# gotaku6629/CTC

Hardware: AMD Instinct MI355X
Metric: ctc_samples_per_sec (higher is better)
Workload: dtype f32; 1 GPU; NoBlankCTC B=256 T=150 C=158 S<=20 fp32 (BASELINE configs[1]); variant=noblank, per_gpu_batch=256, global_batch=256, T=150, C=158, S=20, parallelism=dp1 (batch-sharded), launch=graph, graph_steps=50, step=fused loss+grad launch + scale_grad launch (loss.backward(), grad_out=1)

## Files before the change

### __graft_entry__.py

```python
import os
import sys

ROOT = os.path.dirname(os.path.abspath(__file__))
if ROOT not in sys.path:
    sys.path.insert(0, ROOT)


def build():
    from ctc_amd import build as b
    so = b.build()
    b.build_fault()
    try:
        b.build_host_ext()
    except Exception as e:
        print("build: the optional C++ autograd node was not built (%s: %s)" % (type(e).__name__, str(e).splitlines()[0][:200]))
    b.build_occupant()
    from oracle import ctc_c
    ctc_c.build()
    import ctc_amd
    from ctc_amd import _lib
    _lib.load()
    assert os.path.exists(so) and ctc_amd.SO_PATH == so


def smoke():
    import numpy as np
# ... 23 lines not shown
```

### ctc_amd/csrc/binary.hip

```cpp
#include <cstdlib>
#include <type_traits>

#include "lattice.hpp"
#include "launch.hpp"

namespace ctc {

struct BinaryParams {
    const float *x;
    int64_t st, sb;
    const float *y;
    const int64_t *in_len, *tgt_len;
    int T, B, C, S, SP, CP;
    int stop;
    float loss_scale, grad_scale;
    float *nll, *loss, *grad;
    float *gamma;
    unsigned *counter;
};

constexpr int kBinThreads = 1024;
constexpr int kBinWaves = kBinThreads / kWave;

struct BinarySmem {
    float *em, *al, *be, *dummy, *ys, *drow;
    __device__ BinarySmem(float *base, int T, int SP, int S, int CP)
    {
        em = base + kPrefetch * SP;
        al = em + (size_t)(T + kPrefetch) * SP;
        be = al + (size_t)T * SP;
        dummy = be + (size_t)T * SP;
        ys = dummy + 8;
        drow = ys + (size_t)S * CP;
// ... 939 lines not shown
                         const int64_t *in_len, const int64_t *tgt_len, int T, int B, int C, int S, float loss_scale,
                         float grad_scale, float *nll, float *loss, float *grad, float *gamma, void *workspace,
                         const BinarySwitches &sw)
{
    if (!x || !y || !in_len || !tgt_len || !nll || !(loss || gamma) || !workspace) return CTC_AMD_ERR_BAD_ARGUMENT;
    if (T < 1 || B < 1 || C < 1 || S < 1) return CTC_AMD_ERR_BAD_ARGUMENT;
    p.x = static_cast<const float *>(x);
    p.st = stride_t; p.sb = stride_b; p.y = y;
    p.in_len = in_len; p.tgt_len = tgt_len;
    p.T = T; p.B = B; p.C = C; p.S = S;
    p.stop = sw.stop < 0 ? sw.stop : 0;
    p.loss_scale = loss_scale; p.grad_scale = grad_scale;
    p.nll = nll; p.loss = gamma ? reinterpret_cast<float *>(static_cast<char *>(workspace) + 32) : loss;
    p.grad = gamma ? nullptr : grad; p.gamma = gamma;
    p.counter = static_cast<unsigned *>(workspace);
    return 0;
}

struct BinaryQuery {
    int T, B, C, S, dtype;
    bool want_gamma;
    BinarySwitches sw;
};
enum BinaryFamily { kBinaryUnsupported = 0, kBinaryFlow, kBinaryPipe, kBinaryMfma, kBinaryFused };
struct BinaryPlan {
    int family, K, SP, ch, wt, Tpad, pd, grid;
    size_t lds;
};
static int binary_row_pitch(int C) { return C | 1; }

// ... 25 lines not shown
    BinaryPlan pl = {};
    pl.family = kBinaryFused; pl.K = K; pl.SP = SP; pl.grid = q.B;
    pl.lds = binary_smem_bytes(q.T, SP, q.S, binary_row_pitch(q.C));
    return pl.lds <= kMaxLds ? pl : BinaryPlan{};
}

static int binary_launch(const BinaryPlan &pl, int dtype, BinaryParams &p, hipStream_t s)
{
    const dim3 grid(pl.grid), block(kBinThreads);
    p.SP = pl.SP; p.CP = binary_row_pitch(p.C);
    auto workers = [&](auto wt, auto gamma, auto elem) {
        constexpr bool WT = decltype(wt)::value != 0, GAMMA = decltype(gamma)::value;
        using E = typename decltype(elem)::type;
        if (pl.family == kBinaryFlow)
            return with_constant<1, 2, 3>(pl.ch, [&](auto ch) {
                return launch<binary_flow_kernel<decltype(ch)::value, WT, GAMMA, E>>(grid, block, pl.lds, s, p, pl.pd);
            });
        return with_constant<1, 2, 3, 4>(pl.ch, [&](auto ch) {
            return launch<binary_pipe_kernel<decltype(ch)::value, WT, GAMMA, E>>(grid, block, pl.lds, s, p, pl.pd);
        });
    };
    switch (pl.family) {
        case kBinaryFlow:
        case kBinaryPipe:
            if (p.gamma) return with_logit_elem(dtype, [&](auto elem) { return workers(std::true_type(), std::true_type(), elem); });
            return with_constant<0, 1>(pl.wt, [&](auto wt) { return workers(wt, std::false_type(), LogitElem<float>()); });
        case kBinaryMfma:
            return with_constant<1, 2, 4>(pl.K, [&](auto k) {
                return with_constant<1, 2, 3, 4>(pl.ch, [&](auto ch) {
                    return with_constant<0, 1>(pl.wt, [&](auto wt) {
// ... 62 lines not shown
```

### ctc_amd/csrc/binary_flow.hpp

```cpp
#pragma once

typedef __bf16 bf16x8 __attribute__((ext_vector_type(8)));
typedef unsigned u32x4 __attribute__((ext_vector_type(4)));

#ifndef CTC_FLOW_TILE_WAVES
#define CTC_FLOW_TILE_WAVES 4
#endif
constexpr int kFlowTileWaves = CTC_FLOW_TILE_WAVES;
constexpr int kFlowFirstWorker = 2 + kFlowTileWaves;
constexpr int kFlowWorkers = kBinWaves - kFlowFirstWorker;
constexpr int kFlowRounds = (80 + kFlowWorkers - 1) / kFlowWorkers;
static_assert(kFlowRounds % 2 == 0, "two rounds per gradient group");
constexpr int kFlowGroups = kFlowRounds / 2;
constexpr int kFlowMaxT = 2 * kFlowWorkers * kFlowRounds;
constexpr int kFlowMaxTiles = kFlowMaxT / 16;
constexpr int kFlowFlags = 64;
constexpr int kFlowYRows = (65 + kFlowFirstWorker - 1) / kFlowFirstWorker;

__host__ __device__ inline int flow_yp(int C) { return (C + 31) / 32 * 32 + 8; }
__host__ __device__ inline size_t flow_y_floats(int SP, int C, int PD)
{
    const size_t halfs = (size_t)(SP + 1) * flow_yp(C);
    return (((size_t)SP * PD + 3) & ~(size_t)3) + (((halfs + 1) / 2 + 3) & ~(size_t)3);
}

struct BinaryFlowSmem {
    float *em, *al, *be, *dummy, *q, *zrow, *ys, *dimg;
    unsigned short *y16;
    int *prog, *fail, *tile, *done, *ystage;
    __device__ BinaryFlowSmem(float *base, int T, int SP, int PD, int C)
    {
        em = base + kPrefetch * SP;
        al = em + (size_t)(T + kPrefetch) * SP;
        be = al + (size_t)T * SP;
        dummy = be + (size_t)T * SP;
        int *f = reinterpret_cast<int *>(dummy);
        prog = f + 4;
        fail = f + 6;
        tile = f + 8;
        done = f + 20;
        ystage = f + 32;
        q = dummy + kFlowFlags;
        zrow = q + ((T + 7) & ~3);
        ys = zrow + 64;
        y16 = reinterpret_cast<unsigned short *>(ys + (((size_t)SP * PD + 3) & ~(size_t)3));
        dimg = ys + flow_y_floats(SP, C, PD);
    }
};

static size_t binary_flow_smem_bytes(int T, int SP, int PD, int C)
{
    return ((size_t)(3 * T + 2 * kPrefetch) * SP + kFlowFlags + ((T + 7) & ~3) + 64 + flow_y_floats(SP, C, PD) + (size_t)(T + 1) * PD) * 4;
}

__device__ __forceinline__ void split3_bf16(const float (&f)[8], u32x4 &t0, u32x4 &t1, u32x4 &t2)
{
// ... 78 lines not shown
                for (int j = 0; j < CH; ++j) {
                    const int c = lane + 64 * j;
                    yv[i][j] = (l < p.S && c < p.C) ? yb[l * p.C + c] : 0.f;
                }
            }
        }
    }
    if (tid < kFlowFlags) sm.dummy[tid] = 0.f;
    if (tid >= 128 && tid < 192) sm.zrow[tid - 128] = 0.f;
    for (int i = tid; i < kPrefetch * p.SP; i += kBinThreads) {
        sm.em[i - kPrefetch * p.SP] = kNeg;
        sm.em[p.T * p.SP + i] = kNeg;
    }
    __syncthreads();
    const ScalarLengths lens(p.in_len + b, p.tgt_len + b);

    auto six = [&](const int *f, int equals) -> bool {
        return __builtin_amdgcn_ballot_w64(lane < kFlowFirstWorker && *(lds_cvint *)(f + (lane < kFlowFirstWorker ? lane : 0)) == equals) != 0;
    };
    bool exact = true;
    auto wait_y = [&]() -> bool {
        int spins = 0;
        while (six(sm.ystage, 0)) {
            if (++spins >= (1 << 20)) return false;
            __builtin_amdgcn_s_sleep(1);
        }
        exact = !six(sm.ystage, 2);
        lds_order();
        return true;
    };
// ... 6 lines not shown
#pragma unroll
                for (int j = 0; j < CH; ++j) {
                    const int c = lane + 64 * j;
                    const unsigned bits = __builtin_bit_cast(unsigned, yv[i][j]);
                    inexact = inexact || (bits & 0xffffu) != 0;
                    if (c < YP) sm.y16[l * YP + c] = (unsigned short)(bits >> 16);
                    if (l < p.SP && c < PD) sm.ys[l * PD + c] = yv[i][j];
                }
            }
        }
        lds_order();
        sm.ystage[w] = __builtin_amdgcn_ballot_w64(inexact) == 0 ? 1 : 2;
    }
    int64_t Tb64, L64;
    lens.get(Tb64, L64);
    const bool ok = L64 >= 1 && L64 <= p.S && Tb64 >= L64 && Tb64 <= p.T;
    const int Tb = ok ? (int)Tb64 : 0, L = ok ? (int)L64 : 0;
    const float invC = 1.0f / (float)p.C;
    const float inv2 = invC * kLog2e;
    const float gs = p.grad_scale * invC;
    stamp(p, 1);

    bool starved = false;
    bool have_lse = false;
    float c2 = 0.f;
    const unsigned voff = 4u * lane;
    const int lane_l = lane < p.SP ? lane : 0;
    const bool in_l = lane < L;
    const float ninf = -__builtin_inff();
    int c_tt[kFlowGroups][4], c_tl[kFlowGroups][4], c_hi[kFlowGroups], c_lo[kFlowGroups];
// ... 116 lines not shown
                if (tl[k] >= 0)
                    p.gamma[((int64_t)b * p.T + tl[k]) * p.S + lane] = starved ? __builtin_nanf("") : pe[k] * __builtin_amdgcn_rcpf(sum[k]);
        }
    };
    auto elem = [&](int uu, int jg, unsigned slow4, auto &&P, bool own = false) {
        int tt[4], tl[4], t_hi, t_lo;
        rows_of(uu, jg, tt, tl, t_hi, t_lo, own);
        if (starved) raise_status(p.counter, kStatusBinaryStarved);
        if constexpr (GAMMA) {
#pragma unroll
            for (int i = 0; i < 4; ++i)
                if (tt[i] >= 0 && tl[i] < 0 && lane < p.S) p.gamma[((int64_t)b * p.T + tt[i]) * p.S + lane] = 0.f;
            return;
        }
        lds_order();
        f32x4 acc[CH];
#pragma unroll
        for (int j = 0; j < CH; ++j) acc[j] = f32x4{0.f, 0.f, 0.f, 0.f};
        if (t_hi >= 0) {
            {
                const int ti = tl[lane & 3];
                const float *arow = ti >= 0 ? sm.be + ti * p.SP : sm.zrow;
                const float *yrow = sm.ys + lane;
                auto operands = [&](int l0, float4 &fa, float (&fy)[4][CH]) {
                    fa = *reinterpret_cast<const float4 *>(arow + (l0 < p.SP ? l0 : 0));
#pragma unroll
                    for (int i = 0; i < 4; ++i)
#pragma unroll
                        for (int j = 0; j < CH; ++j) fy[i][j] = yrow[(l0 + i < p.SP ? l0 + i : p.SP - 1) * PD + 64 * j];
                };
// ... 5 lines not shown
                        for (int j = 0; j < CH; ++j) acc[j] = __builtin_amdgcn_mfma_f32_4x4x1f32(fav[i], fy[i][j], acc[j], 0, 0, 0);
                };
                float4 fa0, fa1;
                float fy0[4][CH], fy1[4][CH];
                operands(0, fa0, fy0);
                for (int l0 = 0; l0 < L; l0 += 8) {
                    operands(l0 + 4, fa1, fy1);
                    contract(fa0, fy0);
                    if (l0 + 4 < L) {
                        operands(l0 + 8, fa0, fy0);
                        contract(fa1, fy1);
                    }
                }
            }
        }
        if (!starved && slow4 == 0 && tl[0] >= 0 && tl[1] >= 0 && tl[2] >= 0 && tl[3] >= 0) {
#pragma unroll
            for (int i = 0; i < 4; ++i) {
                float *g = p.grad + ((int64_t)tl[i] * p.B + b) * p.C;
                bin_row_base_settled(g);
#pragma unroll
                for (int j = 0; j < CH; ++j) {
                    const float pr = P(i & 1, i >> 1, j);
                    if (j < CH - 1 || lane + 64 * j < p.C) bin_store_col<WT>(g, voff, j, __builtin_fmaf(pr, gs, -acc[j][i]));
                }
            }
            return;
        }
#pragma unroll
        for (int i = 0; i < 4; ++i) {
            if (tt[i] < 0) continue;
            float *g = p.grad + ((int64_t)tt[i] * p.B + b) * p.C;
            bin_row_base_settled(g);
            const int slot = 2 * (i & 1) + (i >> 1);
            if (tl[i] < 0 || starved) {
                const float fill = starved ? __builtin_nanf("") : 0.f;
#pragma unroll
                for (int j = 0; j < CH; ++j)
                    if (j < CH - 1 || lane + 64 * j < p.C) bin_store_col<WT>(g, voff, j, fill);
            } else if ((slow4 >> slot) & 1) {
#pragma unroll
                for (int j = 0; j < CH; ++j) {
                    const float pr = P(i & 1, i >> 1, j);
                    const float pq = pr * (1.0f - pr);
                    const float gv = __builtin_fmaf(pr, gs, -acc[j][i]) * (pq * __builtin_amdgcn_rcpf(fmaxf(pq, 1e-12f)));
                    if (j < CH - 1 || lane + 64 * j < p.C) bin_store_col<WT>(g, voff, j, gv);
                }
            } else {
#pragma unroll
                for (int j = 0; j < CH; ++j) {
                    const float pr = P(i & 1, i >> 1, j);
                    if (j < CH - 1 || lane + 64 * j < p.C) bin_store_col<WT>(g, voff, j, __builtin_fmaf(pr, gs, -acc[j][i]));
                }
            }
        }
    };

    if (w < 2) {
        if (w == 1 && !p.grad && !GAMMA) return;
        __builtin_amdgcn_s_setprio(3);
        bool starved = false;
        if (Tb > 0) {
            int known = -1;
            auto ready = [&](int i) {
                while (known < i && !starved) {
                    const int t = w == 0 ? known + 1 : Tb - 2 - known;
                    const int m = t >> 4;
// ... 351 lines not shown
```

### ctc_amd/csrc/common.hpp

```cpp
#pragma once
#include <hip/hip_runtime.h>
#include <stdint.h>

#if !defined(CTC_AMD_EXPERIMENTS) &&                                                                            \
    (defined(CTC_X_NOSTATUS) || defined(CTC_X_NOREDUCE) || defined(CTC_X_NORETURN) || defined(CTC_X_NOCHAIN) || \
     defined(CTC_X_NOPRIO) || defined(CTC_X_NOREAD) || defined(CTC_X_NOWRITE) ||                                 \
     defined(CTC_X_WMASK) || defined(CTC_X_NOPROG) || defined(CTC_X_NORENORM) ||                                \
     defined(CTC_X_ROWDPP) || defined(CTC_X_SCALAR_STEP) || defined(CTC_X_NO_POOL_GATHER) || defined(CTC_X_FLOW_NO_GPRIO) || defined(CTC_X_FLOW_NOEXP) || defined(CTC_X_FLOW_NO_DELEGATE) || defined(CTC_X_FLOW_DELEGATE_OWN) || \
     defined(CTC_FLOW_TILE_WAVES))
#error "CTC_X_* experiment switches need -DCTC_AMD_EXPERIMENTS (A/B builds only, never the product library)"
#endif

namespace ctc {

constexpr int kWave = 64;
constexpr float kNeg = -10000000000000.0f;
constexpr float kInfeasible = 1.0e12f;
constexpr float kMasked = -1.0e30f;
__device__ __forceinline__ float masked_floor(float e) { return e < kMasked ? kMasked : e; }

struct LaneStates { int K, SP; };
inline LaneStates lane_states(int S)
{
    int K = 1;
// ... 254 lines not shown

struct ScalarLengths {
    int64_t a, b;
    __device__ __forceinline__ ScalarLengths() : a(0), b(0) {}
    __device__ __forceinline__ ScalarLengths(const int64_t *pa, const int64_t *pb)
    {
        typedef const __attribute__((address_space(4))) int64_t const_i64;
        a = *(const_i64 *)(uintptr_t)pa;
        b = *(const_i64 *)(uintptr_t)pb;
    }
    __device__ __forceinline__ void get(int64_t &va, int64_t &vb) const
    {
        va = a;
        vb = b;
    }
};

__device__ __forceinline__ void bce_logs(float x, float &p, float &lp, float &lq)
{
    p = 1.0f / (1.0f + expf(-x));
    lp = fmaxf(logf(p), -100.0f);
    lq = fmaxf(logf(1.0f - p), -100.0f);
}

template <typename P>
__device__ __forceinline__ void stamp(const P &p, int slot)
{
    if (CTC_DIAG(p) >= 0 || CTC_DIAG(p) <= -100) return;
    if (blockIdx.x == 0 && wave_id() == -CTC_DIAG(p) - 1 && lane_id() == 0) {
        unsigned long long *o = reinterpret_cast<unsigned long long *>(p.counter) + 8 + 2 * slot;
// ... 120 lines not shown
```

### ctc_amd/csrc/launch.hpp

```cpp
#pragma once
#include <hip/hip_runtime.h>

#include <atomic>
#include <cstdlib>
#include <type_traits>

#include "../../include/ctc_amd.h"

namespace ctc {

constexpr size_t kMaxLds = 160 * 1024;
constexpr size_t kDefaultDynLds = 64 * 1024;
constexpr int kMaxDevices = 64;

inline bool within_memory_side_cache(size_t bytes, int T, int B, int C) { return bytes * T * B * C <= ((size_t)230 << 20); }

inline int current_device()
{
    int dev = -1;
    if (hipGetDevice(&dev) != hipSuccess || dev < 0 || dev >= kMaxDevices) return -1;
    return dev;
}

inline int device_cus()
// ... 47 lines not shown
{
    if (smem > kDefaultDynLds) {
        static std::atomic<bool> granted[kMaxDevices];
        const int dev = current_device();
        if (dev < 0 || !granted[dev].load(std::memory_order_relaxed)) {
            hipError_t e = hipFuncSetAttribute(reinterpret_cast<const void *>(kern),
                                               hipFuncAttributeMaxDynamicSharedMemorySize, (int)kMaxLds);
            if (e != hipSuccess) return (int)e;
            if (dev >= 0) granted[dev].store(true, std::memory_order_relaxed);
        }
    }
    hipLaunchKernelGGL(kern, grid, block, smem, stream, args...);
    return (int)hipGetLastError();
}

}
```

### ctc_amd/csrc/noblank.hip

```cpp
#include <type_traits>

#include "lattice.hpp"
#include "launch.hpp"

namespace ctc {

struct NoblankParams {
    const float *x;
    int64_t st, sb;
    const void *lab;
    int lab64;
    const int64_t *in_len, *tgt_len;
    int T, B, C, S, SP;
    int stop;
    float loss_scale, grad_scale;
    float *nll, *loss, *grad;
    float *gamma;
    float *lattice;
    int64_t slab;
    unsigned *counter;
    int next_round;
    float ls_a, ls_b;
    int koff;
};

__device__ __forceinline__ NoblankParams opaque_params(NoblankParams q)
{
#define CTC_OPQ(f) asm volatile("" : "+s"(q.f))
    CTC_OPQ(x); CTC_OPQ(st); CTC_OPQ(sb); CTC_OPQ(lab); CTC_OPQ(lab64); CTC_OPQ(in_len); CTC_OPQ(tgt_len);
    CTC_OPQ(T); CTC_OPQ(B); CTC_OPQ(C); CTC_OPQ(S); CTC_OPQ(SP); CTC_OPQ(stop); CTC_OPQ(loss_scale); CTC_OPQ(grad_scale);
    CTC_OPQ(nll); CTC_OPQ(loss); CTC_OPQ(grad); CTC_OPQ(gamma); CTC_OPQ(lattice); CTC_OPQ(slab); CTC_OPQ(counter);
    CTC_OPQ(next_round); CTC_OPQ(ls_a); CTC_OPQ(ls_b); CTC_OPQ(koff);
#undef CTC_OPQ
    return q;
}

#ifndef CTC_NOBLANK_THREADS
#define CTC_NOBLANK_THREADS 1024
#endif
constexpr int kThreads = CTC_NOBLANK_THREADS;
constexpr int kWaves = kThreads / kWave;
constexpr int kRows = 160 / kWaves;
constexpr int kRowsPerPass = kWaves * kRows;

struct NoblankSmem {
    float *em, *al, *be, *mx, *ls, *dummy;
    int *cnt, *lab, *nxt, *dup, *inv;
// ... 338 lines not shown
    const size_t stride = (size_t)gridDim.x * blockDim.x;
    const size_t i = (size_t)blockIdx.x * blockDim.x + threadIdx.x;
    size_t done = 0;
    if ((reinterpret_cast<uintptr_t>(g) & 7) == 0) {
        wt_u2 *g4 = reinterpret_cast<wt_u2 *>(g);
        const size_t n4 = n / 4;
        const f2_t s2 = {s, s};
        for (size_t k = i; k < n4; k += stride) {
            wt_u2 v = g4[k];
            v.x = r16_narrow2<E>(r16_widen2<E>(v.x) * s2);
            v.y = r16_narrow2<E>(r16_widen2<E>(v.y) * s2);
            g4[k] = v;
        }
        done = n4 * 4;
    }
    for (size_t k = done + i; k < n; k += stride) g[k] = (E)((float)g[k] * s);
}


struct NoblankSwitches {
    bool no_pipe, no_xr, no_r16, no_ps, km;
    bool nograd;
    int stop;
};
static const NoblankSwitches &noblank_switches()
{
    static const NoblankSwitches sw = {diag_env("CTC_AMD_NOPIPE") != 0, diag_env("CTC_AMD_NOXR") != 0,
                                       diag_env("CTC_AMD_NOR16") != 0,  diag_env("CTC_AMD_NOPS") != 0,
                                       diag_env("CTC_AMD_KM") != 0,     diag_env("CTC_AMD_DEBUG_NOGRAD") != 0,
                                       diag_env("CTC_AMD_DEBUG_STOP")};
    return sw;
// ... 10 lines not shown
    const NoblankSizes z = noblank_sizes(T, C, S);
    char *ws = static_cast<char *>(workspace);
    p.x = static_cast<const float *>(x); p.st = stride_t; p.sb = stride_b;
    p.lab = labels; p.lab64 = labels_i64;
    p.in_len = in_len; p.tgt_len = tgt_len;
    p.T = T; p.B = B; p.C = C; p.S = S; p.SP = z.SP;
    p.stop = sw.stop;
    p.loss_scale = loss_scale; p.grad_scale = grad_scale;
    p.nll = nll; p.loss = gamma ? reinterpret_cast<float *>(ws + 32) : loss;
    p.grad = sw.nograd ? nullptr : static_cast<float *>(grad);
    p.gamma = gamma;
    p.counter = static_cast<unsigned *>(workspace);
    p.lattice = z.glb ? reinterpret_cast<float *>(ws + 256 + acc_list_bytes(B)) : nullptr;
    p.slab = z.glb ? (int64_t)noblank_lattice_floats(T, z.SP) : 0;
    p.next_round = 0; p.koff = 0;
    const bool smooth = label_smoothing >= 0.f;
    p.ls_b = smooth ? (1.f - label_smoothing) / (float)C : 0.f;
    p.ls_a = smooth ? label_smoothing - p.ls_b : 1.f;
    return 0;
}

struct NoblankQuery {
    int T, B, C, S;
    int dtype;
    int64_t st, sb;
    unsigned x_low, grad_low;
    bool want_grad, want_gamma, smooth;
    int cus;
    NoblankSwitches sw;
};
// ... 73 lines not shown
}

static int noblank_launch(const NoblankPlan &pl, int dtype, NoblankParams &p, hipStream_t s)
{
    const dim3 grid(pl.grid), block(kThreads);
    p.next_round = pl.next_round; p.koff = pl.koff;
    switch (pl.family) {
        case kNoblankR16:
            return with_row_chunks(pl.n4, pl.n2, [&](auto n4, auto n2) {
                return with_constant<0, 1>(pl.nt, [&](auto nt) {
                    return with_constant<CTC_AMD_BF16, CTC_AMD_F16, CTC_AMD_F32>(dtype, [&](auto dt) {
                        using E = std::conditional_t<decltype(dt)::value == CTC_AMD_BF16, __bf16,
                                                     std::conditional_t<decltype(dt)::value == CTC_AMD_F16, _Float16, float>>;
                        constexpr int A = decltype(n4)::value, Bq = decltype(n2)::value;
                        constexpr bool NT = decltype(nt)::value != 0;
                        if constexpr (4 * A + 2 * Bq <= 12)
                            if (pl.ps) return launch<noblank_r16_kernel<A, Bq, NT, true, E>>(grid, block, pl.lds, s, p);
                        return launch<noblank_r16_kernel<A, Bq, NT, false, E>>(grid, block, pl.lds, s, p);
                    });
                });
            });
#ifdef CTC_AMD_DIAGNOSTICS
        case kNoblankKm:
            return with_row_chunks(pl.n4, pl.n2, [&](auto n4, auto n2) {
                return with_constant<0, 1>(pl.nt, [&](auto nt) {
                    return launch<noblank_km_kernel<decltype(n4)::value, decltype(n2)::value, decltype(nt)::value != 0>>(
                        grid, block, pl.lds, s, p);
                });
            });
#endif
        case kNoblankXr:
        case kNoblankPipelined:
            return with_constant<1, 2, 3, 4>(pl.ch, [&](auto ch) {
// ... 68 lines not shown
                                                  const int64_t *in_len, const int64_t *tgt_len,
                                                  int T, int B, int C, int S, float label_smoothing,
                                                  float loss_scale, float grad_scale,
                                                  float *nll, float *loss, float *grad,
                                                  void *workspace, void *stream)
{
    if (!(label_smoothing >= 0.f && label_smoothing <= 1.f)) return CTC_AMD_ERR_BAD_ARGUMENT;
    return noblank_run(x, stride_t, stride_b, labels, labels_i64, in_len, tgt_len, T, B, C, S, loss_scale, grad_scale,
                       nll, loss, grad, workspace, stream, label_smoothing);
}

extern "C" int ctc_amd_scale_grad(float *grad, const float *grad_out, size_t n, void *stream)
{
    if (!grad || !grad_out) return CTC_AMD_ERR_BAD_ARGUMENT;
    if (n == 0) return 0;
    hipLaunchKernelGGL(scale_grad_kernel, scale_grad_grid(n), dim3(256), 0,
                       static_cast<hipStream_t>(stream), grad, grad_out, n);
    return (int)hipGetLastError();
}

extern "C" int ctc_amd_noblank_loss_grad_typed(const void *x, int x_dtype, int64_t stride_t, int64_t stride_b,
                                               const void *labels, int labels_i64,
                                               const int64_t *in_len, const int64_t *tgt_len,
                                               int T, int B, int C, int S, float label_smoothing,
                                               float loss_scale, float grad_scale,
                                               float *nll, float *loss, void *grad,
                                               void *workspace, void *stream)
{
    if (x_dtype != CTC_AMD_F32 && x_dtype != CTC_AMD_BF16 && x_dtype != CTC_AMD_F16) return CTC_AMD_ERR_BAD_ARGUMENT;
    if (label_smoothing != label_smoothing || label_smoothing > 1.f) return CTC_AMD_ERR_BAD_ARGUMENT;
    return noblank_run(x, stride_t, stride_b, labels, labels_i64, in_len, tgt_len, T, B, C, S, loss_scale, grad_scale,
                       nll, loss, grad, workspace, stream, label_smoothing < 0.f ? -1.f : label_smoothing, x_dtype);
}

extern "C" int ctc_amd_scale_grad_typed(void *grad, int dtype, const float *grad_out, size_t n, void *stream)
{
    if (dtype == CTC_AMD_F32) return ctc_amd_scale_grad(static_cast<float *>(grad), grad_out, n, stream);
    if ((dtype != CTC_AMD_BF16 && dtype != CTC_AMD_F16) || !grad || !grad_out) return CTC_AMD_ERR_BAD_ARGUMENT;
    if (n == 0) return 0;
    if (dtype == CTC_AMD_BF16)
        hipLaunchKernelGGL(scale_grad_lowp_kernel<__bf16>, scale_grad_grid(n), dim3(256), 0,
                           static_cast<hipStream_t>(stream), static_cast<__bf16 *>(grad), grad_out, n);
    else
        hipLaunchKernelGGL(scale_grad_lowp_kernel<_Float16>, scale_grad_grid(n), dim3(256), 0,
                           static_cast<hipStream_t>(stream), static_cast<_Float16 *>(grad), grad_out, n);
    return (int)hipGetLastError();
}

extern "C" int ctc_amd_noblank_posteriors(const float *x, int64_t stride_t, int64_t stride_b,
                                          const void *labels, int labels_i64,
                                          const int64_t *in_len, const int64_t *tgt_len,
                                          int T, int B, int C, int S,
                                          float *nll, float *gamma,
                                          void *workspace, void *stream)
// ... 5 lines not shown

extern "C" int ctc_amd_noblank_posteriors_typed(const void *x, int x_dtype, int64_t stride_t, int64_t stride_b,
                                                const void *labels, int labels_i64,
                                                const int64_t *in_len, const int64_t *tgt_len,
                                                int T, int B, int C, int S,
                                                float *nll, float *gamma,
                                                void *workspace, void *stream)
{
    if (x_dtype != CTC_AMD_F32 && x_dtype != CTC_AMD_BF16 && x_dtype != CTC_AMD_F16) return CTC_AMD_ERR_BAD_ARGUMENT;
    if (!gamma) return CTC_AMD_ERR_BAD_ARGUMENT;
    return noblank_run(x, stride_t, stride_b, labels, labels_i64, in_len, tgt_len, T, B, C, S, 0.f, 0.f, nll, nullptr,
                       nullptr, workspace, stream, -1.f, x_dtype, gamma);
}

#ifdef CTC_AMD_DIAGNOSTICS
extern "C" int ctc_amd_debug_chain_probe(int T, int SP, int waves_alive, int grid, void *out, void *stream, int mode,
                                         int chain_b)
{
    using namespace ctc;
    NoblankParams p = {};
    p.T = T; p.SP = SP; p.S = SP; p.B = grid; p.C = 32;
    p.stop = -77;
    p.counter = reinterpret_cast<unsigned *>(static_cast<unsigned long long *>(out) + 8);
    const size_t smem = r16_smem_bytes(T, SP, 158);
    return launch<r16_chain_probe_kernel>(dim3(grid), dim3(kThreads), smem, static_cast<hipStream_t>(stream), p,
                                          static_cast<unsigned long long *>(out), waves_alive, mode, chain_b);
}

extern "C" int ctc_amd_debug_noblank_plan(int T, int B, int C, int S, int dtype, int64_t stride_t, int64_t stride_b,
                                          unsigned x_low, unsigned grad_low, int want_grad, int want_gamma, int smooth,
// ... 14 lines not shown
```

### ctc_amd/csrc/noblank_r16.hpp

```cpp
#pragma once

namespace ctc {

typedef float f2_t __attribute__((ext_vector_type(2)));

#define CTC_ROW16(OP)                                                                   \
    "s_nop 1\n\t" OP " %0, %0, %0 quad_perm:[1,0,3,2] row_mask:0xf bank_mask:0xf\n\t"   \
    "s_nop 1\n\t" OP " %0, %0, %0 quad_perm:[2,3,0,1] row_mask:0xf bank_mask:0xf\n\t"   \
    "s_nop 1\n\t" OP " %0, %0, %0 row_half_mirror row_mask:0xf bank_mask:0xf\n\t"       \
    "s_nop 1\n\t" OP " %0, %0, %0 row_mirror row_mask:0xf bank_mask:0xf\n\t"            \
    "s_nop 1"
__device__ __forceinline__ void row16_allmax(float &v) { asm volatile(CTC_ROW16("v_max_f32_dpp") : "+v"(v)); }
__device__ __forceinline__ void row16_allsum(float &v) { asm volatile(CTC_ROW16("v_add_f32_dpp") : "+v"(v)); }
__device__ __forceinline__ void row16_allmax(int &v) { asm volatile(CTC_ROW16("v_max_i32_dpp") : "+v"(v)); }

constexpr int kR16Pad = 2 * kPrefetch + 1;
#ifndef CTC_R16_BLOCK
#define CTC_R16_BLOCK 16
#endif
constexpr int kR16Block = CTC_R16_BLOCK;
__host__ __device__ inline int r16_pitch(int T)
{
    int tp = T + 2 * kR16Pad + 1;
    while ((tp & 3) != 2) ++tp;
    return tp;
}

__device__ __forceinline__ int r16_row(int T, int u, int g, int k)
{
    const int H = (T + 1) >> 1, idx = 2 * kPipeWorkers * g + 2 * u + (k >> 1);
    if ((k & 1) == 0) return idx < H ? idx : -1;
    return idx < T - H ? T - 1 - idx : -1;
}

struct R16Smem {
    int TP;
    cell_t *em, *al, *be;
    float *dummy, *stage, *cs;
    int *cnt, *lab, *occ, *done;
    __device__ R16Smem(float *base, int T, int SP, int RP)
    {
        TP = r16_pitch(T);
        cell_t *lat = reinterpret_cast<cell_t *>(base);
        em = lat + kR16Pad;
        al = em + (size_t)(SP + 1) * TP;
        be = al + (size_t)(SP + 1) * TP;
        dummy = reinterpret_cast<float *>(lat + (size_t)3 * (SP + 1) * TP);
        cnt = reinterpret_cast<int *>(dummy + 8);
        lab = cnt + 16;
        occ = lab + ((SP + 3) & ~3);
        cs = reinterpret_cast<float *>(occ + ((SP + 3) & ~3) + 4);
        done = reinterpret_cast<int *>(cs + 4 * kPipeWorkers);
        stage = cs + 64;
    }
};

static size_t r16_smem_bytes(int T, int SP, int C)
{
    const int RP = 32 * ((C + 31) / 32);
    return (size_t)3 * (SP + 1) * r16_pitch(T) * 8 + (8 + 16 + 2 * ((SP + 3) & ~3) + 4 + 64) * 4 +
           (size_t)kPipeWorkers * 4 * RP * 4;
}

template <bool FWD>
__device__ __forceinline__ cell_t r16_chain(const NoblankParams &p, const R16Smem &sm, int T, int Tb, int L, int SP, const int lane)
{
    constexpr int G = kPipeRows / 4;
// ... 320 lines not shown
    {
#pragma unroll
        for (int j = 0; j < N4; ++j) *reinterpret_cast<f4_t *>(trow + off4(j, i16)) = a[j];
#pragma unroll
        for (int k = 0; k < N2; ++k) *reinterpret_cast<f2_t *>(trow + off2(k, i16)) = c[k];
    }
    __device__ static __forceinline__ void zero_tile(float *trow, int i16)
    {
        const f4_t z4 = {0.f, 0.f, 0.f, 0.f};
        const f2_t z2 = {0.f, 0.f};
#pragma unroll
        for (int j = 0; j < N4; ++j) *reinterpret_cast<f4_t *>(trow + off4(j, i16)) = z4;
#pragma unroll
        for (int k = 0; k < N2; ++k) *reinterpret_cast<f2_t *>(trow + off2(k, i16)) = z2;
    }
    template <bool NT, bool LS>
    __device__ __forceinline__ void store_grad(E *g, const float *trow, int i16, float rs, bool col_ok, float cb) const
    {
        const f2_t r2 = {rs, rs}, cb2 = {cb, cb};
        f4_t o4[N4 > 0 ? N4 : 1];
        f2_t o2[N2 > 0 ? N2 : 1];
#pragma unroll
        for (int j = 0; j < N4; ++j) o4[j] = *reinterpret_cast<const f4_t *>(trow + off4(j, i16));
#pragma unroll
        for (int k = 0; k < N2; ++k) o2[k] = *reinterpret_cast<const f2_t *>(trow + off2(k, i16));
#pragma unroll
        for (int j = 0; j < N4; ++j) {
            const f4_t o = o4[j];
            f2_t olo = {o.x, o.y}, ohi = {o.z, o.w};
            if (LS) { olo += cb2; ohi += cb2; }
            const f2_t xlo = {a[j].x, a[j].y}, xhi = {a[j].z, a[j].w};
            const f2_t vlo = __builtin_elementwise_fma(xlo, r2, olo), vhi = __builtin_elementwise_fma(xhi, r2, ohi);
            if (!(kLast4 && j == N4 - 1) || col_ok) {
                if constexpr (kLowp) {
                    const wt_u2 n = {r16_narrow2<E>(vlo), r16_narrow2<E>(vhi)};
                    grad_store<NT, wt_u2, 4>(reinterpret_cast<wt_u2 *>(g + off4(j, i16)), n);
                } else {
                    const f4_t v = {vlo.x, vlo.y, vhi.x, vhi.y};
                    grad_store<NT>(reinterpret_cast<f4_t *>(g + off4(j, i16)), v);
                }
            }
        }
#pragma unroll
        for (int k = 0; k < N2; ++k) {
            f2_t o = o2[k];
            if (LS) o += cb2;
            const f2_t v = __builtin_elementwise_fma(c[k], r2, o);
            if (k < N2 - 1 || col_ok) {
                if constexpr (kLowp) grad_store<NT, unsigned, 4>(reinterpret_cast<unsigned *>(g + off2(k, i16)), r16_narrow2<E>(v));
                else grad_store<NT>(reinterpret_cast<f2_t *>(g + off2(k, i16)), v);
            }
        }
    }
    __device__ __forceinline__ void touch() const
    {
        if constexpr (kLowp) {
#pragma unroll
            for (int j = 0; j < N4; ++j) asm volatile("" ::"v"(this->ra[j]));
#pragma unroll
            for (int k = 0; k < N2; ++k) asm volatile("" ::"v"(this->rc[k]));
        } else {
#pragma unroll
            for (int j = 0; j < N4; ++j) asm volatile("" ::"v"(a[j]));
#pragma unroll
            for (int k = 0; k < N2; ++k) asm volatile("" ::"v"(c[k]));
        }
    }
    template <bool NT>
    __device__ static __forceinline__ void store_zero(E *g, int i16, bool col_ok)
    {
        if constexpr (kLowp) {
            const wt_u2 z4 = {0u, 0u};
#pragma unroll
            for (int j = 0; j < N4; ++j)
                if (!(kLast4 && j == N4 - 1) || col_ok) grad_store<NT, wt_u2, 4>(reinterpret_cast<wt_u2 *>(g + off4(j, i16)), z4);
#pragma unroll
            for (int k = 0; k < N2; ++k)
                if (k < N2 - 1 || col_ok) grad_store<NT, unsigned, 4>(reinterpret_cast<unsigned *>(g + off2(k, i16)), 0u);
            return;
        }
        const f4_t z4 = {0.f, 0.f, 0.f, 0.f};
        const f2_t z2 = {0.f, 0.f};
#pragma unroll
        for (int j = 0; j < N4; ++j)
            if (!(kLast4 && j == N4 - 1) || col_ok) grad_store<NT>(reinterpret_cast<f4_t *>(g + off4(j, i16)), z4);
#pragma unroll
        for (int k = 0; k < N2; ++k)
            if (k < N2 - 1 || col_ok) grad_store<NT>(reinterpret_cast<f2_t *>(g + off2(k, i16)), z2);
    }
};

static bool r16_shape(int C, int &n4, int &n2)
{
    if (C < 2 || C > 256 || (C & 1)) return false;
    const int U = (C + 31) / 32;
    if (U & 1) { n4 = U / 2; n2 = 1; }
    else if ((C & 3) == 0) { n4 = U / 2; n2 = 0; }
// ... 23 lines not shown

    if (CTC_DIAG(p) == 1) return;
    stamp(p, 0);
    stamp_setup(p, 0);
    auto spread = [&](int which) {
        if (CTC_DIAG(p) != -50 || w != 1 || lane != 0) return;
        const int bid = blockIdx.x, nb = gridDim.x;
        const int slot = bid == 0 ? 0 : bid == nb / 2 ? 2 : bid == nb - 1 ? 4 : -1;
        if (slot < 0) return;
        unsigned long long *o = reinterpret_cast<unsigned long long *>(p.counter) + 8 + 2 * (slot + which);
        o[0] = __builtin_amdgcn_s_memtime();
        o[1] = __builtin_amdgcn_s_memrealtime();
    };
    spread(0);
    ScalarLengths len(p.in_len + b, p.tgt_len + b);
    int tv0[G];
    Row v[G];
#ifdef CTC_R16_NX
    constexpr int NX = PS ? CTC_R16_NX : 0;
#else
    constexpr int NX = PS ? (NT ? 2 : 3) : 0;
#endif
    Row nx[NX > 0 ? NX : 1];
    const bool col_ok = Row::off_last(i16) < p.C;
    const int c_last = col_ok ? Row::off_last(i16) : p.C - (Row::kLast4 ? 4 : 2);
    const int Hh = (p.T + 1) >> 1;
    bool grp[G];
#pragma unroll
    for (int g = 0; g < G; ++g) grp[g] = u >= 0 && 2 * kPipeWorkers * g + 2 * u < Hh;
    int klab = 0;
// ... 118 lines not shown
    int tv[G];
#pragma unroll
    for (int g = 0; g < G; ++g) tv[g] = PS ? opaque_v(tv0[g]) : tv0[g];
    const bool has_grad = PS || p.grad != nullptr, has_gamma = !PS && p.gamma != nullptr;
    auto load_next = [&]() {
        if (!PS) return;
#pragma unroll
        for (int g = 0; g < NX; ++g) nx[g].load(r16_xrow<E>(p, tv[g] >= 0 ? tv[g] : 0, bn), i16, c_last);
    };
#define CTC_R16_RELOAD(g)                                                                             \
    do {                                                                                              \
        if (PS && (g) >= NX) v[g].load(r16_xrow<E>(p, tv[g] >= 0 ? tv[g] : 0, bn), i16, c_last); \
    } while (0)
    if (!PS && Tb == 0) {
        if (p.grad) {
#pragma unroll
            for (int g = 0; g < G; ++g)
                if (tv[g] >= 0) Row::template store_zero<NT>(reinterpret_cast<E *>(p.grad) + ((int64_t)tv[g] * p.B + b) * p.C, i16, col_ok);
        }
        if (p.gamma) {
#pragma unroll
            for (int g = 0; g < G; ++g)
                for (int l = i16; l < p.S && tv[g] >= 0; l += 16) p.gamma[((int64_t)b * p.T + tv[g]) * p.S + l] = 0.f;
        }
        return;
    }
    float *tile = sm.stage + (size_t)u * 4 * RP;
    float *trow = tile + rho * RP;
    int lst[2];
    float *gat[2];
#pragma unroll
    for (int s = 0; s < 2; ++s) {
        lst[s] = 16 * s + i16;
// ... 145 lines not shown
    bool have_ref = false;
    int occn[2] = {0, 0}, max_occ = 0;
    if (has_grad) {
        int spins = 0;
        while (*(lds_cvint *)(sm.occ + ((p.SP + 3) & ~3) + 1) == 0) {
            if (++spins >= kSpinLimit) { starved = true; break; }
            __builtin_amdgcn_s_sleep(2);
        }
        lds_order();
        occn[0] = own[0] ? sm.occ[lst[0]] : 0;
        occn[1] = own[1] ? sm.occ[lst[1]] : 0;
        max_occ = __builtin_amdgcn_readfirstlane(sm.occ[(p.SP + 3) & ~3]);
    }
    const bool first_occ[2] = {own[0] && occn[0] == 0, own[1] && occn[1] == 0};
    float *const sink = sm.dummy + 4;
#pragma unroll
    for (int g = G - 1; g >= 0; --g) {
        if (!grp[g]) continue;
        const int need_a = need_a_[g], need_b = need_b_[g];
        if (need_a > 0) {
            int spins = 0;
            while (*(lds_cvint *)(sm.cnt + kPipeWorkers) < need_a || *(lds_cvint *)(sm.cnt + kPipeWorkers + 1) < need_b) {
                if (++spins >= kSpinLimit) { starved = true; break; }
                __builtin_amdgcn_s_sleep(8);
            }
            lds_order();
        }
#ifdef CTC_AMD_FAULT_INJECT
        if (b == 1) starved = true;
#endif
// ... 34 lines not shown
            rinv = __builtin_nanf("");
            raise_status(p.counter, kStatusNoblankStarved);
        }
#pragma unroll
        for (int s = 0; s < 2; ++s) *(first_occ[s] ? gat[s] : sink) = z[s] * rinv;
        for (int k = 1; k <= max_occ; ++k) {
            lds_order();
#pragma unroll
            for (int s = 0; s < 2; ++s)
                if (own[s] && occn[s] == k) *gat[s] += z[s] * rinv;
        }
        lds_order();
        if (t >= 0) {
            E *gp = grow[g];
            const bool mass = !live || tot > 0.f;
            if (smooth) x.template store_grad<NT, true>(gp, trow, i16, live && mass ? rs[g] * (1.f - p.ls_b) : 0.f, col_ok, live && mass ? -p.ls_b * gsc : 0.f);
            else x.template store_grad<NT, false>(gp, trow, i16, mass ? rs[g] : 0.f, col_ok, 0.f);
        }
        lds_order();
#pragma unroll
        for (int s = 0; s < 2; ++s) *(own[s] ? gat[s] : sink) = 0.f;
        lds_order();
        CTC_R16_RELOAD(g);
    }
    stamp(p, 7);
    spread(1);
#undef CTC_R16_RELOAD
    };

    if (u < 0) {
        for (;;) {
// ... 75 lines not shown
```

Measured before the change: 19.22 million samples/s.

## Fold scale_grad into captured loss kernel node by patching upstream pointer

During graph capture, the loss kernel launch is recorded, and when the following scale_grad call targets the same grad buffer it rewrites the captured kernel node's params to carry an upstream grad_out pointer instead of launching a separate scale kernel. The kernels read the upstream scalar and multiply gradients in-kernel, taking a fast path when it equals 1. This removes one kernel launch and a full read-modify-write pass over the T*B*C gradient tensor per step. It adds host-side bookkeeping and relies on graph node param mutation, and changes rounding order for low-precision dtypes.

```diff
diff --git a/__graft_entry__.py b/__graft_entry__.py
--- a/__graft_entry__.py
+++ b/__graft_entry__.py
@@ -10,6 +10,7 @@
     from ctc_amd import build as b
     so = b.build()
     b.build_fault()
+    b.build_diag()
     try:
         b.build_host_ext()
     except Exception as e:
diff --git a/ctc_amd/csrc/binary.hip b/ctc_amd/csrc/binary.hip
--- a/ctc_amd/csrc/binary.hip
+++ b/ctc_amd/csrc/binary.hip
@@ -17,6 +17,7 @@
     float *nll, *loss, *grad;
     float *gamma;
     unsigned *counter;
+    const float *upstream;
 };
 
 constexpr int kBinThreads = 1024;
@@ -986,6 +987,7 @@
     p.nll = nll; p.loss = gamma ? reinterpret_cast<float *>(static_cast<char *>(workspace) + 32) : loss;
     p.grad = gamma ? nullptr : grad; p.gamma = gamma;
     p.counter = static_cast<unsigned *>(workspace);
+    p.upstream = nullptr;
     return 0;
 }
 
@@ -1041,6 +1043,9 @@
         using E = typename decltype(elem)::type;
         if (pl.family == kBinaryFlow)
             return with_constant<1, 2, 3>(pl.ch, [&](auto ch) {
+                if constexpr (!GAMMA)
+                    return launch_loss<binary_flow_kernel<decltype(ch)::value, WT, GAMMA, E>>(
+                        grid, block, pl.lds, s, true, CTC_AMD_F32, (size_t)p.T * p.B * p.C, p, pl.pd);
                 return launch<binary_flow_kernel<decltype(ch)::value, WT, GAMMA, E>>(grid, block, pl.lds, s, p, pl.pd);
             });
         return with_constant<1, 2, 3, 4>(pl.ch, [&](auto ch) {
diff --git a/ctc_amd/csrc/binary_flow.hpp b/ctc_amd/csrc/binary_flow.hpp
--- a/ctc_amd/csrc/binary_flow.hpp
+++ b/ctc_amd/csrc/binary_flow.hpp
@@ -25,7 +25,7 @@
 }
 
 struct BinaryFlowSmem {
-    float *em, *al, *be, *dummy, *q, *zrow, *ys, *dimg;
+    float *em, *al, *be, *dummy, *q, *zrow, *ys, *dimg, *up;
     unsigned short *y16;
     int *prog, *fail, *tile, *done, *ystage;
     __device__ BinaryFlowSmem(float *base, int T, int SP, int PD, int C)
@@ -40,6 +40,7 @@
         tile = f + 8;
         done = f + 20;
         ystage = f + 32;
+        up = dummy + 40;
         q = dummy + kFlowFlags;
         zrow = q + ((T + 7) & ~3);
         ys = zrow + 64;
@@ -148,6 +149,7 @@
     }
     __syncthreads();
     const ScalarLengths lens(p.in_len + b, p.tgt_len + b);
+    const ScalarUpstream upstream(GAMMA ? nullptr : p.upstream);
 
     auto six = [&](const int *f, int equals) -> bool {
         return __builtin_amdgcn_ballot_w64(lane < kFlowFirstWorker && *(lds_cvint *)(f + (lane < kFlowFirstWorker ? lane : 0)) == equals) != 0;
@@ -184,6 +186,7 @@
     }
     int64_t Tb64, L64;
     lens.get(Tb64, L64);
+    if (!GAMMA) sm.up[w] = upstream.value();
     const bool ok = L64 >= 1 && L64 <= p.S && Tb64 >= L64 && Tb64 <= p.T;
     const int Tb = ok ? (int)Tb64 : 0, L = ok ? (int)L64 : 0;
     const float invC = 1.0f / (float)p.C;
@@ -330,6 +333,8 @@
             return;
         }
         lds_order();
+        const float go = __builtin_bit_cast(float, __builtin_amdgcn_readfirstlane(__builtin_bit_cast(int, sm.up[w])));
+        const bool scaled = __builtin_bit_cast(unsigned, go) != 0x3f800000u;
         f32x4 acc[CH];
 #pragma unroll
         for (int j = 0; j < CH; ++j) acc[j] = f32x4{0.f, 0.f, 0.f, 0.f};
@@ -365,7 +370,7 @@
                 }
             }
         }
-        if (!starved && slow4 == 0 && tl[0] >= 0 && tl[1] >= 0 && tl[2] >= 0 && tl[3] >= 0) {
+        if (!scaled && !starved && slow4 == 0 && tl[0] >= 0 && tl[1] >= 0 && tl[2] >= 0 && tl[3] >= 0) {
 #pragma unroll
             for (int i = 0; i < 4; ++i) {
                 float *g = p.grad + ((int64_t)tl[i] * p.B + b) * p.C;
@@ -385,7 +390,8 @@
             bin_row_base_settled(g);
             const int slot = 2 * (i & 1) + (i >> 1);
             if (tl[i] < 0 || starved) {
-                const float fill = starved ? __builtin_nanf("") : 0.f;
+                float fill = starved ? __builtin_nanf("") : 0.f;
+                if (scaled) fill *= go;
 #pragma unroll
                 for (int j = 0; j < CH; ++j)
                     if (j < CH - 1 || lane + 64 * j < p.C) bin_store_col<WT>(g, voff, j, fill);
@@ -394,14 +400,17 @@
                 for (int j = 0; j < CH; ++j) {
                     const float pr = P(i & 1, i >> 1, j);
                     const float pq = pr * (1.0f - pr);
-                    const float gv = __builtin_fmaf(pr, gs, -acc[j][i]) * (pq * __builtin_amdgcn_rcpf(fmaxf(pq, 1e-12f)));
+                    float gv = __builtin_fmaf(pr, gs, -acc[j][i]) * (pq * __builtin_amdgcn_rcpf(fmaxf(pq, 1e-12f)));
+                    if (scaled) gv *= go;
                     if (j < CH - 1 || lane + 64 * j < p.C) bin_store_col<WT>(g, voff, j, gv);
                 }
             } else {
 #pragma unroll
                 for (int j = 0; j < CH; ++j) {
                     const float pr = P(i & 1, i >> 1, j);
-                    if (j < CH - 1 || lane + 64 * j < p.C) bin_store_col<WT>(g, voff, j, __builtin_fmaf(pr, gs, -acc[j][i]));
+                    float gv = __builtin_fmaf(pr, gs, -acc[j][i]);
+                    if (scaled) gv *= go;
+                    if (j < CH - 1 || lane + 64 * j < p.C) bin_store_col<WT>(g, voff, j, gv);
                 }
             }
         }
diff --git a/ctc_amd/csrc/common.hpp b/ctc_amd/csrc/common.hpp
--- a/ctc_amd/csrc/common.hpp
+++ b/ctc_amd/csrc/common.hpp
@@ -292,6 +292,17 @@
         va = a;
         vb = b;
     }
+};
+
+static __device__ const float kUnitUpstream = 1.0f;
+struct ScalarUpstream {
+    float v;
+    __device__ __forceinline__ explicit ScalarUpstream(const float *up)
+    {
+        typedef const __attribute__((address_space(4))) float const_f32;
+        v = *(const_f32 *)(uintptr_t)(up ? up : &kUnitUpstream);
+    }
+    __device__ __forceinline__ float value() const { return v; }
 };
 
 __device__ __forceinline__ void bce_logs(float x, float &p, float &lp, float &lq)
diff --git a/ctc_amd/csrc/launch.hpp b/ctc_amd/csrc/launch.hpp
--- a/ctc_amd/csrc/launch.hpp
+++ b/ctc_amd/csrc/launch.hpp
@@ -2,7 +2,10 @@
 #include <hip/hip_runtime.h>
 
 #include <atomic>
+#include <cstddef>
 #include <cstdlib>
+#include <cstring>
+#include <mutex>
 #include <type_traits>
 
 #include "../../include/ctc_amd.h"
@@ -85,4 +88,147 @@
     return (int)hipGetLastError();
 }
 
-}
+#pragma GCC visibility push(hidden)
+constexpr int kFoldRecords = 16;
+constexpr size_t kFoldParamBytes = 256;
+
+struct FoldRecord {
+    bool live, consumed, foldable;
+    hipStream_t stream;
+    unsigned long long capture_id;
+    hipGraphNode_t node;
+    void *func;
+    dim3 grid, block;
+    unsigned lds;
+    alignas(16) unsigned char params[kFoldParamBytes];
+    size_t upstream_offset;
+    int extra, n_extra;
+    const void *grad;
+    size_t n;
+    int dtype;
+};
+struct FoldTable {
+    std::mutex lock;
+    FoldRecord rec[kFoldRecords];
+    unsigned next_victim;
+    std::atomic<unsigned> taken, refused;
+};
+inline FoldTable &fold_table()
+{
+    static FoldTable t;
+    return t;
+}
+
+inline bool captured_tail(hipStream_t stream, unsigned long long &id, hipGraphNode_t &node)
+{
+    hipStreamCaptureStatus st = hipStreamCaptureStatusNone;
+    hipGraph_t graph = nullptr;
+    const hipGraphNode_t *deps = nullptr;
+    size_t ndeps = 0;
+    id = 0;
+    if (hipStreamGetCaptureInfo_v2(stream, &st, &id, &graph, &deps, &ndeps) != hipSuccess) {
+        (void)hipGetLastError();
+        return false;
+    }
+    if (st != hipStreamCaptureStatusActive || ndeps != 1 || !deps) return false;
+    node = deps[0];
+    return true;
+}
+
+template <auto kern, typename P, typename... Extra>
+inline void note_loss_launch(dim3 grid, dim3 block, size_t smem, hipStream_t stream, const P &p, bool foldable,
+                             const void *grad, size_t n, int dtype, Extra... extra)
+{
+    static_assert(sizeof(P) <= kFoldParamBytes && std::is_trivially_copyable<P>::value, "params copy");
+    static_assert(sizeof...(Extra) <= 1, "one trailing int at most");
+    hipStreamCaptureStatus st = hipStreamCaptureStatusNone;
+    if (hipStreamIsCapturing(stream, &st) != hipSuccess) {
+        (void)hipGetLastError();
+        return;
+    }
+    FoldTable &t = fold_table();
+    std::lock_guard<std::mutex> guard(t.lock);
+    FoldRecord *r = nullptr;
+    for (FoldRecord &q : t.rec)
+        if (q.live && q.stream == stream) r = &q;
+    if (st != hipStreamCaptureStatusActive) {
+        if (r) r->live = false;
+        return;
+    }
+    unsigned long long id;
+    hipGraphNode_t node;
+    if (!captured_tail(stream, id, node)) {
+        if (r) r->live = false;
+        return;
+    }
+    if (!r)
+        for (FoldRecord &q : t.rec)
+            if (!q.live) { r = &q; break; }
+    if (!r) r = &t.rec[t.next_victim++ % kFoldRecords];
+    r->live = true; r->consumed = false; r->foldable = foldable;
+    r->stream = stream; r->capture_id = id; r->node = node;
+    r->func = reinterpret_cast<void *>(kern);
+    r->grid = grid; r->block = block; r->lds = (unsigned)smem;
+    memcpy(r->params, &p, sizeof(P));
+    r->upstream_offset = offsetof(P, upstream);
+    r->n_extra = (int)sizeof...(Extra);
+    r->extra = 0;
+    ((r->extra = extra), ...);
+    r->grad = grad; r->n = n; r->dtype = dtype;
+}
+
+inline bool fold_scale_grad(hipStream_t stream, const void *grad, int dtype, const float *grad_out, size_t n)
+{
+    FoldTable &t = fold_table();
+    std::lock_guard<std::mutex> guard(t.lock);
+    FoldRecord *r = nullptr;
+    for (FoldRecord &q : t.rec)
+        if (q.live && q.stream == stream) r = &q;
+    if (!r) return false;
+    unsigned long long id;
+    hipGraphNode_t node;
+    hipStreamCaptureStatus st = hipStreamCaptureStatusNone;
+    if (hipStreamIsCapturing(stream, &st) != hipSuccess) (void)hipGetLastError();
+    if (st != hipStreamCaptureStatusActive) {
+        r->live = false;
+        return false;
+    }
+    bool ok = captured_tail(stream, id, node) && id == r->capture_id && node == r->node &&
+              r->foldable && !r->consumed && grad == r->grad && n == r->n && dtype == r->dtype;
+    if (ok) {
+        memcpy(r->params + r->upstream_offset, &grad_out, sizeof(grad_out));
+        void *args[2] = {r->params, &r->extra};
+        hipKernelNodeParams np = {};
+        np.func = r->func;
+        np.gridDim = r->grid;
+        np.blockDim = r->block;
+        np.sharedMemBytes = r->lds;
+        np.kernelParams = args;
+        np.extra = nullptr;
+        if (hipGraphKernelNodeSetParams(r->node, &np) != hipSuccess) {
+            (void)hipGetLastError();
+            const float *none = nullptr;
+            memcpy(r->params + r->upstream_offset, &none, sizeof(none));
+            ok = false;
+        }
+    }
+    if (ok) {
+        r->consumed = true;
+        t.taken.fetch_add(1, std::memory_order_relaxed);
+    } else {
+        t.refused.fetch_add(1, std::memory_order_relaxed);
+    }
+    return ok;
+}
+
+template <auto kern, typename P, typename... Extra>
+inline int launch_loss(dim3 grid, dim3 block, size_t smem, hipStream_t stream, bool foldable, int dtype, size_t n, const P &p,
+                       Extra... extra)
+{
+    const int rc = launch<kern>(grid, block, smem, stream, p, extra...);
+    if (rc == 0 && p.grad) note_loss_launch<kern>(grid, block, smem, stream, p, foldable, p.grad, n, dtype, extra...);
+    return rc;
+}
+#pragma GCC visibility pop
+
+}
diff --git a/ctc_amd/csrc/noblank.hip b/ctc_amd/csrc/noblank.hip
--- a/ctc_amd/csrc/noblank.hip
+++ b/ctc_amd/csrc/noblank.hip
@@ -22,6 +22,7 @@
     int next_round;
     float ls_a, ls_b;
     int koff;
+    const float *upstream;
 };
 
 __device__ __forceinline__ NoblankParams opaque_params(NoblankParams q)
@@ -30,7 +31,7 @@
     CTC_OPQ(x); CTC_OPQ(st); CTC_OPQ(sb); CTC_OPQ(lab); CTC_OPQ(lab64); CTC_OPQ(in_len); CTC_OPQ(tgt_len);
     CTC_OPQ(T); CTC_OPQ(B); CTC_OPQ(C); CTC_OPQ(S); CTC_OPQ(SP); CTC_OPQ(stop); CTC_OPQ(loss_scale); CTC_OPQ(grad_scale);
     CTC_OPQ(nll); CTC_OPQ(loss); CTC_OPQ(grad); CTC_OPQ(gamma); CTC_OPQ(lattice); CTC_OPQ(slab); CTC_OPQ(counter);
-    CTC_OPQ(next_round); CTC_OPQ(ls_a); CTC_OPQ(ls_b); CTC_OPQ(koff);
+    CTC_OPQ(next_round); CTC_OPQ(ls_a); CTC_OPQ(ls_b); CTC_OPQ(koff); CTC_OPQ(upstream);
 #undef CTC_OPQ
     return q;
 }
@@ -399,7 +400,11 @@
         }
         done = n4 * 4;
     }
-    for (size_t k = done + i; k < n; k += stride) g[k] = (E)((float)g[k] * s);
+    for (size_t k = done + i; k < n; k += stride) {
+        const unsigned short e = *reinterpret_cast<const unsigned short *>(g + k);
+        const f2_t v = r16_widen2<E>((unsigned)e) * f2_t{s, s};
+        *reinterpret_cast<unsigned short *>(g + k) = (unsigned short)r16_narrow2<E>(v);
+    }
 }
 
 
@@ -440,6 +445,7 @@
     p.lattice = z.glb ? reinterpret_cast<float *>(ws + 256 + acc_list_bytes(B)) : nullptr;
     p.slab = z.glb ? (int64_t)noblank_lattice_floats(T, z.SP) : 0;
     p.next_round = 0; p.koff = 0;
+    p.upstream = nullptr;
     const bool smooth = label_smoothing >= 0.f;
     p.ls_b = smooth ? (1.f - label_smoothing) / (float)C : 0.f;
     p.ls_a = smooth ? label_smoothing - p.ls_b : 1.f;
@@ -543,9 +549,11 @@
                                                      std::conditional_t<decltype(dt)::value == CTC_AMD_F16, _Float16, float>>;
                         constexpr int A = decltype(n4)::value, Bq = decltype(n2)::value;
                         constexpr bool NT = decltype(nt)::value != 0;
+                        const size_t n = (size_t)p.T * p.B * p.C;
                         if constexpr (4 * A + 2 * Bq <= 12)
-                            if (pl.ps) return launch<noblank_r16_kernel<A, Bq, NT, true, E>>(grid, block, pl.lds, s, p);
-                        return launch<noblank_r16_kernel<A, Bq, NT, false, E>>(grid, block, pl.lds, s, p);
+                            if (pl.ps)
+                                return launch_loss<noblank_r16_kernel<A, Bq, NT, true, E>>(grid, block, pl.lds, s, !p.gamma, dtype, n, p);
+                        return launch_loss<noblank_r16_kernel<A, Bq, NT, false, E>>(grid, block, pl.lds, s, !p.gamma, dtype, n, p);
                     });
                 });
             });
@@ -644,6 +652,7 @@
 {
     if (!grad || !grad_out) return CTC_AMD_ERR_BAD_ARGUMENT;
     if (n == 0) return 0;
+    if (fold_scale_grad(static_cast<hipStream_t>(stream), grad, CTC_AMD_F32, grad_out, n)) return 0;
     hipLaunchKernelGGL(scale_grad_kernel, scale_grad_grid(n), dim3(256), 0,
                        static_cast<hipStream_t>(stream), grad, grad_out, n);
     return (int)hipGetLastError();
@@ -668,6 +677,7 @@
     if (dtype == CTC_AMD_F32) return ctc_amd_scale_grad(static_cast<float *>(grad), grad_out, n, stream);
     if ((dtype != CTC_AMD_BF16 && dtype != CTC_AMD_F16) || !grad || !grad_out) return CTC_AMD_ERR_BAD_ARGUMENT;
     if (n == 0) return 0;
+    if (fold_scale_grad(static_cast<hipStream_t>(stream), grad, dtype, grad_out, n)) return 0;
     if (dtype == CTC_AMD_BF16)
         hipLaunchKernelGGL(scale_grad_lowp_kernel<__bf16>, scale_grad_grid(n), dim3(256), 0,
                            static_cast<hipStream_t>(stream), static_cast<__bf16 *>(grad), grad_out, n);
@@ -703,6 +713,14 @@
 }
 
 #ifdef CTC_AMD_DIAGNOSTICS
+extern "C" int ctc_amd_debug_scale_folds(unsigned *taken, unsigned *refused)
+{
+    if (!taken || !refused) return CTC_AMD_ERR_BAD_ARGUMENT;
+    *taken = ctc::fold_table().taken.load(std::memory_order_relaxed);
+    *refused = ctc::fold_table().refused.load(std::memory_order_relaxed);
+    return 0;
+}
+
 extern "C" int ctc_amd_debug_chain_probe(int T, int SP, int waves_alive, int grid, void *out, void *stream, int mode,
                                          int chain_b)
 {
diff --git a/ctc_amd/csrc/noblank_r16.hpp b/ctc_amd/csrc/noblank_r16.hpp
--- a/ctc_amd/csrc/noblank_r16.hpp
+++ b/ctc_amd/csrc/noblank_r16.hpp
@@ -36,7 +36,7 @@
 struct R16Smem {
     int TP;
     cell_t *em, *al, *be;
-    float *dummy, *stage, *cs;
+    float *dummy, *stage, *cs, *up;
     int *cnt, *lab, *occ, *done;
     __device__ R16Smem(float *base, int T, int SP, int RP)
     {
@@ -51,6 +51,7 @@
         occ = lab + ((SP + 3) & ~3);
         cs = reinterpret_cast<float *>(occ + ((SP + 3) & ~3) + 4);
         done = reinterpret_cast<int *>(cs + 4 * kPipeWorkers);
+        up = cs + 4 * kPipeWorkers + 4;
         stage = cs + 64;
     }
 };
@@ -401,23 +402,39 @@
 #pragma unroll
         for (int k = 0; k < N2; ++k) *reinterpret_cast<f2_t *>(trow + off2(k, i16)) = z2;
     }
-    template <bool NT, bool LS>
-    __device__ __forceinline__ void store_grad(E *g, const float *trow, int i16, float rs, bool col_ok, float cb) const
+    template <bool NT, bool LS, bool SC = false>
+    __device__ __forceinline__ void store_grad(E *g, const float *trow, int i16, float rs, bool col_ok, float cb, float go = 1.f) const
     {
         const f2_t r2 = {rs, rs}, cb2 = {cb, cb};
+        auto times_go = [&](float a) {
+            float r;
+            asm("v_mul_f32 %0, %1, %2" : "=v"(r) : "s"(go), "v"(a));
+            return r;
+        };
+        auto scaled = [&](f2_t v) {
+            if constexpr (!SC) {
+                return v;
+            } else {
+                if constexpr (kLowp) v = r16_widen2<E>(r16_narrow2<E>(v));
+                return f2_t{times_go(v.x), times_go(v.y)};
+            }
+        };
         f4_t o4[N4 > 0 ? N4 : 1];
         f2_t o2[N2 > 0 ? N2 : 1];
-#pragma unroll
-        for (int j = 0; j < N4; ++j) o4[j] = *reinterpret_cast<const f4_t *>(trow + off4(j, i16));
-#pragma unroll
-        for (int k = 0; k < N2; ++k) o2[k] = *reinterpret_cast<const f2_t *>(trow + off2(k, i16));
+        if constexpr (!SC) {
+#pragma unroll
+            for (int j = 0; j < N4; ++j) o4[j] = *reinterpret_cast<const f4_t *>(trow + off4(j, i16));
+#pragma unroll
+            for (int k = 0; k < N2; ++k) o2[k] = *reinterpret_cast<const f2_t *>(trow + off2(k, i16));
+        }
 #pragma unroll
         for (int j = 0; j < N4; ++j) {
+            if constexpr (SC) o4[j] = *reinterpret_cast<const f4_t *>(trow + off4(j, i16));
             const f4_t o = o4[j];
             f2_t olo = {o.x, o.y}, ohi = {o.z, o.w};
             if (LS) { olo += cb2; ohi += cb2; }
             const f2_t xlo = {a[j].x, a[j].y}, xhi = {a[j].z, a[j].w};
-            const f2_t vlo = __builtin_elementwise_fma(xlo, r2, olo), vhi = __builtin_elementwise_fma(xhi, r2, ohi);
+            const f2_t vlo = scaled(__builtin_elementwise_fma(xlo, r2, olo)), vhi = scaled(__builtin_elementwise_fma(xhi, r2, ohi));
             if (!(kLast4 && j == N4 - 1) || col_ok) {
                 if constexpr (kLowp) {
                     const wt_u2 n = {r16_narrow2<E>(vlo), r16_narrow2<E>(vhi)};
@@ -430,9 +447,10 @@
         }
 #pragma unroll
         for (int k = 0; k < N2; ++k) {
+            if constexpr (SC) o2[k] = *reinterpret_cast<const f2_t *>(trow + off2(k, i16));
             f2_t o = o2[k];
             if (LS) o += cb2;
-            const f2_t v = __builtin_elementwise_fma(c[k], r2, o);
+            const f2_t v = scaled(__builtin_elementwise_fma(c[k], r2, o));
             if (k < N2 - 1 || col_ok) {
                 if constexpr (kLowp) grad_store<NT, unsigned, 4>(reinterpret_cast<unsigned *>(g + off2(k, i16)), r16_narrow2<E>(v));
                 else grad_store<NT>(reinterpret_cast<f2_t *>(g + off2(k, i16)), v);
@@ -454,20 +472,21 @@
         }
     }
     template <bool NT>
-    __device__ static __forceinline__ void store_zero(E *g, int i16, bool col_ok)
+    __device__ static __forceinline__ void store_zero(E *g, int i16, bool col_ok, float zv = 0.f)
     {
         if constexpr (kLowp) {
-            const wt_u2 z4 = {0u, 0u};
+            const unsigned z = r16_narrow2<E>(f2_t{zv, zv});
+            const wt_u2 z4 = {z, z};
 #pragma unroll
             for (int j = 0; j < N4; ++j)
                 if (!(kLast4 && j == N4 - 1) || col_ok) grad_store<NT, wt_u2, 4>(reinterpret_cast<wt_u2 *>(g + off4(j, i16)), z4);
 #pragma unroll
             for (int k = 0; k < N2; ++k)
-                if (k < N2 - 1 || col_ok) grad_store<NT, unsigned, 4>(reinterpret_cast<unsigned *>(g + off2(k, i16)), 0u);
+                if (k < N2 - 1 || col_ok) grad_store<NT, unsigned, 4>(reinterpret_cast<unsigned *>(g + off2(k, i16)), z);
             return;
         }
-        const f4_t z4 = {0.f, 0.f, 0.f, 0.f};
-        const f2_t z2 = {0.f, 0.f};
+        const f4_t z4 = {zv, zv, zv, zv};
+        const f2_t z2 = {zv, zv};
 #pragma unroll
         for (int j = 0; j < N4; ++j)
             if (!(kLast4 && j == N4 - 1) || col_ok) grad_store<NT>(reinterpret_cast<f4_t *>(g + off4(j, i16)), z4);
@@ -521,6 +540,7 @@
     };
     spread(0);
     ScalarLengths len(p.in_len + b, p.tgt_len + b);
+    if (w == kChainB) *sm.up = ScalarUpstream(p.upstream).value();
     int tv0[G];
     Row v[G];
 #ifdef CTC_R16_NX
@@ -669,9 +689,11 @@
     } while (0)
     if (!PS && Tb == 0) {
         if (p.grad) {
+            const float go = *sm.up;
+            const float zv = go != 1.0f ? 0.f * go : 0.f;
 #pragma unroll
             for (int g = 0; g < G; ++g)
-                if (tv[g] >= 0) Row::template store_zero<NT>(reinterpret_cast<E *>(p.grad) + ((int64_t)tv[g] * p.B + b) * p.C, i16, col_ok);
+                if (tv[g] >= 0) Row::template store_zero<NT>(reinterpret_cast<E *>(p.grad) + ((int64_t)tv[g] * p.B + b) * p.C, i16, col_ok, zv);
         }
         if (p.gamma) {
 #pragma unroll
@@ -847,6 +869,7 @@
     }
     const bool first_occ[2] = {own[0] && occn[0] == 0, own[1] && occn[1] == 0};
     float *const sink = sm.dummy + 4;
+    const unsigned go_bits = __builtin_amdgcn_readfirstlane(__builtin_bit_cast(unsigned, *sm.up));
 #pragma unroll
     for (int g = G - 1; g >= 0; --g) {
         if (!grp[g]) continue;
@@ -911,7 +934,11 @@
         if (t >= 0) {
             E *gp = grow[g];
             const bool mass = !live || tot > 0.f;
-            if (smooth) x.template store_grad<NT, true>(gp, trow, i16, live && mass ? rs[g] * (1.f - p.ls_b) : 0.f, col_ok, live && mass ? -p.ls_b * gsc : 0.f);
+            if (go_bits != 0x3f800000u) {
+                const float go = __builtin_bit_cast(float, go_bits);
+                if (smooth) x.template store_grad<NT, true, true>(gp, trow, i16, live && mass ? rs[g] * (1.f - p.ls_b) : 0.f, col_ok, live && mass ? -p.ls_b * gsc : 0.f, go);
+                else x.template store_grad<NT, false, true>(gp, trow, i16, mass ? rs[g] : 0.f, col_ok, 0.f, go);
+            } else if (smooth) x.template store_grad<NT, true>(gp, trow, i16, live && mass ? rs[g] * (1.f - p.ls_b) : 0.f, col_ok, live && mass ? -p.ls_b * gsc : 0.f);
             else x.template store_grad<NT, false>(gp, trow, i16, mass ? rs[g] : 0.f, col_ok, 0.f);
         }
         lds_order();
```

Measured after the change: 21.62 million samples/s, median of 6. 1.13x the previous value.
